# calebhabesh/NM03-Capstone-Project

Hardware: AMD Instinct MI355X
Metric: DICOM slices/sec through full pipeline (T1+C cohort) at 1/2/4/8 MI355X (higher is better)
Workload: dtype fp32

## Files before the change

### include/nm03/engine.h

```cpp
#pragma once

#include <cstdint>
#include <functional>
#include <memory>
#include <string>
#include <vector>

#include "nm03/golden.h"
#include "nm03/params.h"

namespace nm03 {

struct WorkItem {
  std::string path;
  std::string out_dir;
};

enum SliceCode : int32_t {
  kSliceOk = 0,
  kSliceLoadError = 1,
  kSliceTooSmall = 2,
  kSliceDeviceError = 3,
  kSliceExportError = 4,
  kSliceNotRun = 5,
};

struct SliceStatus {
  int32_t code = kSliceNotRun;
  std::string message;
};

struct StageTimes {
  double load_s = 0;
  double h2d_s = 0;
  double kernels_s = 0;
  double write_s = 0;
  double load_cpu_s = 0;
  double write_cpu_s = 0;
  double slot_cpu_s = 0;
  double wall_s = 0;
  int64_t batches = 0, slices_ok = 0, slices_failed = 0;
  int64_t bytes_in = 0, bytes_out = 0;
  int64_t jpeg_fallbacks = 0;
};

struct EngineConfig {
  int device = 0;
  int batch_size = 25;
  int streams = 3;
  int threads = 16;
  std::vector<int> cpus;
  int max_dim = 512;
  PipelineParams pipe;
  RenderParams render;
  bool export_jpeg = true;
  bool resume = false;
  bool host_only = false;
  uint32_t jpeg_out_cap = 0;
  bool shared_stream = false;
  int pack_slack = -1;
  int upload_chunk_kb = -1;
  int create_writers = 4;
  bool lazy_slots = false;
};

// ... 46 lines not shown
```

### include/nm03/gpu_types.h

```cpp
#pragma once

#include <cstdint>

namespace nm03::gpu {

inline constexpr int kMedTileW = 64, kMedTileH = 64;
inline constexpr int kShpTileW = 64, kShpTileH = 64;
inline constexpr int kSrgMaxDim = 512;
inline constexpr int kMaxSliceDim = 4096;

constexpr uint32_t xcd_tile(uint32_t b, uint32_t n) {
  const uint32_t x = b & 7u, k = b >> 3, q = n >> 3, r = n & 7u;
  return (x < r ? x * (q + 1u) : r * (q + 1u) + (x - r) * q) + k;
}

struct SliceDesc {
  uint32_t raw_off;
  uint32_t mask_off;
  uint16_t w, h;
  uint16_t wpr;
  uint8_t type;
  uint8_t stored_bits;
  float slope, intercept;
  uint32_t seed_off;
  uint16_t seed_count;
  uint16_t flags;
  uint32_t f32_off;
  uint32_t med_tile0;
  uint32_t blob_off;
  uint32_t lut_off;
  uint32_t lut_base;
};
static_assert(sizeof(SliceDesc) == 52, "SliceDesc layout");
inline constexpr uint32_t kNoLut = 0xFFFFFFFFu;
inline constexpr uint16_t kSliceFlagPacked12 = 1;

struct TileDesc {
  uint32_t slice;
  uint16_t tx, ty;
};

struct SeedXY {
  int16_t x, y;
};

struct SliceStats {
  uint32_t key_min, key_max;
  uint32_t s_min, s_max;
};

struct PipeConsts {
  float nmin, nmax, nlow, nhigh, cmin, cmax;
  float gain;
  float band_lo, band_hi;
  float taps[16];
  int mask_radius;
  int median_k;
  int connectivity;
// ... 45 lines not shown
```

### include/nm03/pack12.h

```cpp
#pragma once

#include <cstddef>
#include <cstdint>

namespace nm03::pack12 {

bool available();

size_t pack(const uint16_t* src, size_t n, uint8_t* dst);

bool fits12(const uint16_t* src, size_t n);

void pack_stream(const uint16_t* src, size_t n, uint8_t* dst);

bool pack_stream_checked(const uint16_t* src, size_t n, uint8_t* dst);

void unpack(const uint8_t* src, size_t n, uint16_t* dst);

}
```

### src/io/pack12.cpp

```cpp
#include "nm03/pack12.h"

#include <immintrin.h>

#include <cstdlib>
#include <cstring>

#include "nm03/dicom.h"

namespace nm03::pack12 {

namespace {

__attribute__((target("avx2"))) size_t pack_avx2(const uint16_t* src, size_t n, uint8_t* dst) {
  __m256i acc = _mm256_setzero_si256();
  for (size_t i = 0; i < n; i += 16) acc = _mm256_or_si256(acc, _mm256_loadu_si256(reinterpret_cast<const __m256i*>(src + i)));
  if (!_mm256_testz_si256(acc, _mm256_set1_epi16((short)0xF000))) return 0;
  const __m256i lo_mask = _mm256_set1_epi32(0x00000FFF), hi_mask = _mm256_set1_epi32(0x00FFF000);
  const __m256i shuf = _mm256_setr_epi8(0, 1, 2, 4, 5, 6, 8, 9, 10, 12, 13, 14, -1, -1, -1, -1,
                                        0, 1, 2, 4, 5, 6, 8, 9, 10, 12, 13, 14, -1, -1, -1, -1);
  uint8_t* d = dst;
  for (size_t i = 0; i < n; i += 16, d += 24) {
    const __m256i v = _mm256_loadu_si256(reinterpret_cast<const __m256i*>(src + i));
    const __m256i p = _mm256_or_si256(_mm256_and_si256(v, lo_mask), _mm256_and_si256(_mm256_srli_epi32(v, 4), hi_mask));
    const __m256i c = _mm256_shuffle_epi8(p, shuf);
// ... 60 lines not shown
    }
    if (m32 < m) {
      acc = _mm512_or_si512(acc, _mm512_zextsi256_si512(_mm256_loadu_si256(reinterpret_cast<const __m256i*>(src + i + m32))));
      pack16(src + i + m32, bounce + m32 / 2 * 3);
    }
    bounce_out(dst + i / 2 * 3, bounce, m / 2 * 3);
  }
  _mm_sfence();
  return _mm512_test_epi16_mask(acc, _mm512_set1_epi16((short)0xF000)) == 0;
}

bool use_avx512() {
  static const bool ok = [] {
    return __builtin_cpu_supports("avx512f") && __builtin_cpu_supports("avx512bw") &&
           __builtin_cpu_supports("avx512vbmi");
  }();
  return ok;
}

bool pack_stream_any(const uint16_t* src, size_t n, uint8_t* dst) {
  return use_avx512() ? pack_stream_avx512(src, n, dst) : pack_stream_avx2(src, n, dst);
}

}

bool fits12(const uint16_t* src, size_t n) { return n && !(n & 15) && available() && fits_avx2(src, n); }

void pack_stream(const uint16_t* src, size_t n, uint8_t* dst) { (void)pack_stream_any(src, n, dst); }

bool pack_stream_checked(const uint16_t* src, size_t n, uint8_t* dst) {
  return n && !(n & 15) && available() && pack_stream_any(src, n, dst);
}

bool available() {
  static const bool ok = __builtin_cpu_supports("avx2");
  return ok;
}

size_t pack(const uint16_t* src, size_t n, uint8_t* dst) {
  if (n == 0 || (n & 15) || !available()) return 0;
  return pack_avx2(src, n, dst);
}

void unpack(const uint8_t* src, size_t n, uint16_t* dst) {
  for (size_t k = 0; 2 * k < n; ++k) {
    const uint32_t v = (uint32_t)src[3 * k] | ((uint32_t)src[3 * k + 1] << 8) | ((uint32_t)src[3 * k + 2] << 16);
// ... 7 lines not shown
```

### src/kernels/k1_median.hip

```cpp
#include <hip/hip_runtime.h>

#include <cstdlib>

#include "device_util.h"
#include "nm03/gpu_types.h"
#include "nm03/kernels.h"
#include "nm03/pixel_math.h"

namespace nm03::gpu {
using nm03::gpu::vmax;
using nm03::gpu::vmin;
#include "nm03/median_net.inc"

template <int K>
__device__ __forceinline__ void run_net(const uint32_t* P, int stride, int r, int g, u16x2* out) {
  auto ld = [&](int rr, int cc) -> u16x2 { return as_u16x2(P[(r + rr) * stride + 8 * g + cc]); };
  if constexpr (K == 3) median_net_k3_w8_h1<u16x2>(ld, out);
  else if constexpr (K == 5) median_net_k5_w8_h1<u16x2>(ld, out);
  else if constexpr (K == 7) median_net_k7_w8_h1<u16x2>(ld, out);
  else median_net_k9_w8_h1<u16x2>(ld, out);
}

template <int K>
__global__ __launch_bounds__(256) __attribute__((amdgpu_waves_per_eu(K <= 7 ? 4 : 2))) void median_kernel(const uint16_t* __restrict__ raw, uint16_t* __restrict__ med,
                                                     const SliceDesc* __restrict__ descs,
                                                     const TileDesc* __restrict__ tiles, SliceStats* stats,
                                                     uint32_t* __restrict__ tile_mm, int dbg,
                                                     const uint16_t* __restrict__ blob, uint16_t* __restrict__ raw_out) {
  constexpr int R = K / 2;
  constexpr int PW = 32 + K - 1;
  constexpr int PS = PW | 1;
  constexpr int PR = 64 + K - 1;
  __shared__ uint32_t P[PR * PS];

  const TileDesc t = tiles[blockIdx.x];
  const SliceDesc d = descs[t.slice];
  const int x0 = t.tx * kMedTileW, y0 = t.ty * kMedTileH;
  const int W = d.w, H = d.h;
  const bool from_blob = blob != nullptr;
  const bool packed = from_blob && (d.flags & kSliceFlagPacked12);
  const uint16_t* src = from_blob ? blob + d.blob_off : raw + d.raw_off;
  const uint8_t* pb = reinterpret_cast<const uint8_t*>(src);
  auto sample = [&](int y, int x) -> uint16_t {
    const uint32_t p = (uint32_t)y * W + x;
    if (!packed) return src[p];
    const uint32_t o = (3u * p) >> 1;
    const uint32_t v = (uint32_t)pb[o] | ((uint32_t)pb[o + 1] << 8);
    return (uint16_t)((p & 1u) ? (v >> 4) : (v & 0xFFFu));
  };
  uint16_t* rdst = from_blob ? raw_out + d.raw_off : nullptr;
  const int yin_hi = min(y0 + kMedTileH, H), xin_hi = min(x0 + kMedTileW, W);

  uint32_t kmin = 0xFFFFu, kmax = 0u;
  const uint32_t ksb = d.stored_bits;
  const uint32_t km = d.type == kI16 ? 1u << (ksb - 1u) : 0u, kc = d.type == kI16 ? 0x8000u - km : 0u;
  auto key_pair = [&](uint32_t lo, uint32_t hi) -> uint32_t {
    const uint32_t a = (__builtin_amdgcn_ubfe(lo, 0u, ksb) ^ km) + kc;
    const uint32_t b = (__builtin_amdgcn_ubfe(hi, 0u, ksb) ^ km) + kc;
    return __builtin_amdgcn_perm(b, a, 0x05040100u);
  };
  u16x2 pmin = as_u16x2(0xFFFFFFFFu), pmax = as_u16x2(0u);
  if ((W & 3) == 0 && (d.raw_off & 3) == 0 && (!from_blob || packed || (d.blob_off & 3) == 0)) {
    constexpr int NT = (PR * 10 + 255) / 256;
    uint2 ld[NT][2];
#pragma unroll
    for (int t = 0; t < NT; ++t) {
      const int i = threadIdx.x + 256 * t;
      if (i >= PR * 10) break;
      const int r = i / 10, gi = i - r * 10;
      const int y = clampi(y0 - R + r, 0, H - 1);
#pragma unroll
      for (int h = 0; h < 2; ++h) {
        const int xs = clampi(x0 - 4 + 4 * (gi + 8 * h), 0, W - 4);
        if (packed) {
          const size_t o = ((size_t)y * W + xs) * 3 >> 1;
          ld[t][h] = *reinterpret_cast<const uint2*>(pb + (o & ~(size_t)3));
        } else {
          ld[t][h] = *reinterpret_cast<const uint2*>(src + (size_t)y * W + xs);
        }
      }
    }
#pragma unroll
    for (int t = 0; t < NT; ++t) {
      const int i = threadIdx.x + 256 * t;
      if (i >= PR * 10) break;
      const int r = i / 10, gi = i - r * 10;
      const int yy = y0 - R + r;
      const int y = clampi(yy, 0, H - 1);
      const bool row_in = rdst && yy >= y0 && yy < yin_hi;
      uint16_t px[2][4];
#pragma unroll
      for (int h = 0; h < 2; ++h) {
        const int g4 = gi + 8 * h;
        const int xs = x0 - 4 + 4 * g4;
        uint2 v = ld[t][h];
        if (packed) {
          const size_t o = ((size_t)y * W + clampi(xs, 0, W - 4)) * 3 >> 1;
          const uint64_t b = ((uint64_t)v.x | ((uint64_t)v.y << 32)) >> ((o & 2) * 8);
          v.x = ((uint32_t)b & 0xFFFu) | (((uint32_t)(b >> 12) & 0xFFFu) << 16);
          v.y = ((uint32_t)(b >> 24) & 0xFFFu) | (((uint32_t)(b >> 36) & 0xFFFu) << 16);
        }
        px[h][0] = (uint16_t)v.x;
        px[h][1] = (uint16_t)(v.x >> 16);
        px[h][2] = (uint16_t)v.y;
        px[h][3] = (uint16_t)(v.y >> 16);
        if (xs < 0) px[h][1] = px[h][2] = px[h][3] = px[h][0];
        if (xs >= W) px[h][0] = px[h][1] = px[h][2] = px[h][3];
        const bool store = h == 0 ? gi >= 1 : (g4 >= 10 && g4 <= 16);
        if (store && row_in && xs >= x0 && xs < xin_hi) {
          typedef unsigned int u32x2 __attribute__((ext_vector_type(2)));
          __builtin_nontemporal_store(u32x2{v.x, v.y}, reinterpret_cast<u32x2*>(rdst + (size_t)yy * W + xs));
        }
      }
#pragma unroll
      for (int q = 0; q < 4; ++q) {
        const int c = 4 * gi + q - (4 - R);
        if (c < 0 || c >= PW) continue;
        const uint32_t kp = key_pair(px[0][q], px[1][q]);
        P[r * PS + c] = kp;
// ... 111 lines not shown
```

### src/python/bindings.cpp

```cpp
#include <hip/hip_runtime_api.h>
#include <pybind11/functional.h>
#include <pybind11/numpy.h>
#include <pybind11/pybind11.h>
#include <pybind11/stl.h>

#include <sys/mman.h>
#include <unistd.h>

#include <algorithm>
#include <chrono>
#include <cstring>
#include <mutex>
#include <thread>
#include <vector>

#include "nm03/app.h"
#include "nm03/cohort.h"
#include "nm03/comm.h"
#include "nm03/cpu_sampler.h"
#include "nm03/dicom.h"
#include "nm03/engine.h"
#include "nm03/metaimage.h"
#include "nm03/numa.h"
#include "nm03/golden.h"
#include "nm03/jpeg.h"
#include "nm03/jpeg_dct.h"
#include "nm03/jpeg_lossless.h"
#include "nm03/kernels.h"
#include "nm03/synth.h"
#include "nm03/volume.h"
#include "nm03/volume_slabs.h"

namespace py = pybind11;
using namespace nm03;

namespace {

template <class T>
py::array_t<T> to_np(const std::vector<T>& v, std::vector<py::ssize_t> shape) {
  py::array_t<T> a(shape);
  std::memcpy(a.mutable_data(), v.data(), v.size() * sizeof(T));
  return a;
}

template <class T>
std::vector<T> from_np(const py::array_t<T, py::array::c_style | py::array::forcecast>& a) {
// ... 489 lines not shown
        s.rows = rows;
        s.cols = cols;
        s.seed = seed;
        s.threads = threads;
        s.test_slice = test_slice;
        s.decoy_series = decoy;
        s.type = signed_px ? kI16 : kU16;
        py::gil_scoped_release nogil;
        return synth::generate_cohort(s);
      },
      py::arg("data_root"), py::arg("patients") = 20, py::arg("min_slices") = 21, py::arg("max_slices") = 25,
      py::arg("rows") = 256, py::arg("cols") = 256, py::arg("seed") = 20250404, py::arg("threads") = 8,
      py::arg("test_slice") = true, py::arg("decoy") = false, py::arg("signed") = false);
  m.def("synth_flat", [](const std::string& root, int count, int rows, int cols, uint64_t seed, int threads) {
    py::gil_scoped_release nogil;
    return synth::generate_flat(root, count, rows, cols, seed, threads);
  });
  m.def("phantom_slice", [](int rows, int cols, int patient, int slice, int nslices, uint64_t seed) {
    std::vector<uint16_t> v((size_t)rows * cols);
    synth::phantom_slice(rows, cols, patient, slice, nslices, seed, v.data());
    return to_np<uint16_t>(v, {rows, cols});
  });

  m.def(
      "golden_run",
      [](py::array_t<uint16_t, py::array::c_style | py::array::forcecast> raw, const std::string& type, int stored_bits,
         float slope, float intercept, const PipelineParams& p, const RenderParams& rp, float sx, float sy) {
        golden::SliceInput s = slice_from(raw, type, stored_bits, slope, intercept, sx, sy);
        golden::SliceResult r = golden::run(s, p, true);
        py::dict d;
        d["clipped"] = to_np<float>(r.clipped, {s.h, s.w});
        d["median"] = to_np<float>(r.median, {s.h, s.w});
        d["sharpened"] = to_np<float>(r.sharpened, {s.h, s.w});
        d["band"] = mask2d(r.band, s.h, s.w);
        d["region"] = mask2d(r.region, s.h, s.w);
        d["eroded"] = mask2d(r.eroded, s.h, s.w);
        d["dilated"] = mask2d(r.dilated, s.h, s.w);
        d["window"] = py::make_tuple(r.window_lo, r.window_hi);
        golden::SliceJpegs j = golden::export_jpegs(s, r, p, rp);
        d["jpeg_original"] = py::bytes((const char*)j.original.data(), j.original.size());
        d["jpeg_processed"] = py::bytes((const char*)j.processed.data(), j.processed.size());
        if (rp.overlay) {
          d["overlay"] = to_np<uint8_t>(j.overlay_canvas, {rp.out_height, rp.out_width, 3});
          d["jpeg_overlay"] = py::bytes((const char*)j.overlay.data(), j.overlay.size());
        }
        return d;
// ... 158 lines not shown
            }
            return w;
          },
          py::arg("data_root"), py::arg("out_root"), py::arg("reaper") = nullptr);
  struct Ticket {
    RunTicket t;
  };
  py::class_<Ticket>(m, "RunTicket");
  auto times_dict = [](const StageTimes& t) {
    py::dict td;
    td["load_s"] = t.load_s;
    td["h2d_s"] = t.h2d_s;
    td["kernels_s"] = t.kernels_s;
    td["write_s"] = t.write_s;
    td["load_cpu_s"] = t.load_cpu_s;
    td["write_cpu_s"] = t.write_cpu_s;
    td["slot_cpu_s"] = t.slot_cpu_s;
    td["wall_s"] = t.wall_s;
    td["batches"] = t.batches;
    td["slices_ok"] = t.slices_ok;
    td["slices_failed"] = t.slices_failed;
    td["bytes_in"] = t.bytes_in;
    td["bytes_out"] = t.bytes_out;
    td["jpeg_fallbacks"] = t.jpeg_fallbacks;
    return td;
  };
  auto compact = [times_dict](const std::vector<SliceStatus>& st, const StageTimes& t) {
    py::array_t<int32_t> codes((py::ssize_t)st.size());
    auto c = codes.mutable_unchecked<1>();
    py::dict msgs;
    for (size_t i = 0; i < st.size(); ++i) {
      c((py::ssize_t)i) = st[i].code;
      if (st[i].code != kSliceOk) msgs[py::int_(i)] = st[i].message;
    }
    return py::make_tuple(codes, msgs, times_dict(t));
  };
  py::class_<Engine>(m, "Engine")
      .def(py::init<const EngineConfig&>())
      .def(
          "run",
          [times_dict](Engine& e, const std::vector<std::pair<std::string, std::string>>& items) {
            std::vector<WorkItem> wi;
            for (auto& p : items) wi.push_back({p.first, p.second});
            StageTimes t;
            std::vector<SliceStatus> st;
            {
// ... 765 lines not shown
```

### src/runtime/engine.cpp

```cpp
#include "nm03/engine.h"

#include <hip/hip_runtime_api.h>
#include <fcntl.h>
#include <linux/capability.h>
#include <signal.h>
#include <sys/mman.h>
#include <sys/prctl.h>
#include <sys/resource.h>
#include <sys/syscall.h>
#include <unistd.h>

#include <algorithm>
#include <ctime>
#include <atomic>
#include <array>
#include <chrono>
#include <condition_variable>
#include <cstdlib>
#include <cstring>
#include <deque>
#include <unordered_map>
#include <mutex>
#include <tuple>
#include <thread>
// ... 17 lines not shown
namespace {

constexpr size_t kAlign = 256;
inline size_t align_up(size_t v, size_t a) { return (v + a - 1) / a * a; }
inline int64_t thread_cpu_ns() {
  timespec ts;
  clock_gettime(CLOCK_THREAD_CPUTIME_ID, &ts);
  return (int64_t)ts.tv_sec * 1000000000 + ts.tv_nsec;
}

inline double now_s() {
  return std::chrono::duration<double>(std::chrono::steady_clock::now().time_since_epoch()).count();
}

enum Plane { kPBand = 0, kPRegion, kPDilated, kPEroded, kPBorderR, kPBorderE, kPBorderD, kNumPlanes };

struct LoadedSlice {
  bool ok = false;
  int w = 0, h = 0;
  uint8_t type = kU16, stored_bits = 16;
  float slope = 1.f, intercept = 0.f, sx = 1.f, sy = 1.f;
  uint32_t blob_off = 0;
  bool packed = false;
};


struct Slot {
  hipStream_t stream = nullptr;
  hipEvent_t ev0 = nullptr, ev1 = nullptr, ev2 = nullptr;
  hipStream_t up = nullptr;
  bool owns_stream = true;
  int cap_slices = 0, cap_canvases = 0;
  size_t cap_pixels = 0;
  size_t hole_slack = 0;
  std::atomic<size_t> hole_credit{0};
  size_t off_stats = 0, off_desc = 0, off_medt = 0, off_shpt = 0, off_seeds = 0, off_render = 0, off_jpeg = 0,
         raw_base = 0, blob_bytes = 0;
  size_t max_medt = 0, max_shpt = 0;
  uint8_t* h_blob = nullptr;
  uint8_t* raw_cpu = nullptr;
  uint8_t* h_single = nullptr;
  size_t single_bytes = 0;
  uint8_t* d_blob = nullptr;
  uint16_t* d_raw_x = nullptr;
  uint16_t* d_med = nullptr;
  uint32_t* d_tile_mm = nullptr;
// ... 127 lines not shown
  }
  hipStream_t s = nullptr;
  check_hip(hipStreamCreateWithFlags(&s, hipStreamNonBlocking), what);
  return s;
}

template <class T>
T* dmalloc(size_t count, const char* what) {
  void* p = nullptr;
  check_hip(hipMalloc(&p, std::max<size_t>(count, 1) * sizeof(T)), what);
  return (T*)p;
}

}

struct Engine::Impl {
  EngineConfig cfg;
  numa::Placement place;
  std::unique_ptr<ThreadPool> pool;
  std::vector<std::unique_ptr<Slot>> slots;
  std::vector<uint8_t> jpeg_header;
  int32_t divs[64];
  PipeConsts pc{};
  bool pack12_ = pack12::available();
  uint32_t out_cap_ = 0;
  bool host_only_ = false;
  std::vector<uint8_t> tmpl_[2];

  explicit Impl(const EngineConfig& c) : cfg(c), place(c.device, c.cpus) {
    if (const char* e = std::getenv("NM03_PACK12"); e && *e && *e == '0') pack12_ = false;
    out_cap_ = cfg.jpeg_out_cap ? std::max<uint32_t>(64, cfg.jpeg_out_cap)
                                : (uint32_t)std::max<size_t>(32 * 1024, (size_t)cfg.render.out_width * cfg.render.out_height * 3 / 8) + 64;
    out_cap_ = (out_cap_ + 15u) & ~15u;
    overlay_ = cfg.render.overlay;
    if (overlay_ && cfg.host_only)
      throw std::invalid_argument("overlay is rendered and encoded on the GPU: not available with host_only");
    if (overlay_ && cfg.render.jpeg_sampling == jpeg::kSamplingGray)
      throw std::invalid_argument("overlay needs a YCbCr JPEG layout (jpeg_sampling 0 or 1): a gray file cannot carry colour");
    ov_cap_ = cfg.jpeg_out_cap ? out_cap_ : (2 * (out_cap_ - 64) + 64 + 15u) & ~15u;
    ov_color_ = (uint32_t)cfg.render.overlay_color[0] | ((uint32_t)cfg.render.overlay_color[1] << 8) |
                ((uint32_t)cfg.render.overlay_color[2] << 16);
    upload_chunk_ = cfg.upload_chunk_kb < 0 ? (size_t)2 << 20 : (size_t)cfg.upload_chunk_kb << 10;
    host_only_ = cfg.host_only;
    if (host_only_) upload_chunk_ = 0;
    if (cfg.batch_size < 1) cfg.batch_size = 1;
    if (cfg.streams < 1) cfg.streams = 1;
    if (cfg.max_dim < 16) cfg.max_dim = 16;
    if (cfg.max_dim > kMaxSliceDim) throw DeviceError("max_dim above " + std::to_string(kMaxSliceDim) + " not supported");
    const auto& p = cfg.pipe;
    if (p.median_window != 3 && p.median_window != 5 && p.median_window != 7 && p.median_window != 9)
      throw DeviceError("median window must be 3, 5, 7 or 9");
    if (p.sharpen_mask < 1 || p.sharpen_mask > 15 || !(p.sharpen_mask & 1))
      throw DeviceError("sharpen mask must be odd and ≤ 15");
// ... 398 lines not shown
        if (e == hipSuccess) return;
        if (e != hipErrorNotReady) check_hip(e, "batch sync");
        if (now_s() > until) break;
        for (int k = 0; k < 32; ++k) __builtin_ia32_pause();
      }
    }
    const double scale = (double)std::max(1, nslices);
    const double target = 0.8 * s.batch_ema_s * scale;
    for (;;) {
      const hipError_t e = hipEventQuery(ev);
      if (e == hipSuccess) break;
      if (e != hipErrorNotReady) check_hip(e, "batch sync");
      const double ahead = target - (now_s() - t_enq);
      if (ahead > 100e-6)
        std::this_thread::sleep_for(std::chrono::duration<double>(std::min(ahead, 250e-6)));
      else
        std::this_thread::sleep_for(std::chrono::microseconds(20));
    }
    const double took = (now_s() - t_enq) / scale;
    s.batch_ema_s = s.batch_ema_s > 0 ? 0.75 * s.batch_ema_s + 0.25 * took : took;
  }

  void load_into(Slot& s, int i, size_t item, const std::string& path, SliceStatus& st, std::atomic<int64_t>& load_ns,
                 std::atomic<int64_t>& bytes_in) {
    thread_local std::vector<uint8_t> buf;
    TraceRange tr("nm03.load");
    const double t0 = now_s();
    try {
      if (fault_plan().corrupt_dicom == (int64_t)item) throw SliceError("injected fault: corrupt DICOM data");
      dicom::SliceFile file(AT_FDCWD, path.c_str(), path, dicom::ReadMode::kStaged);
      const dicom::Header& h = file.header(buf);
      const int frame = dicom::select_frame(h, cfg.pipe.frame);
      const size_t n = file.size();
      const int md = cfg.pipe.min_dim;
      if (md > 0 && (h.cols < md || h.rows < md)) {
        st.code = kSliceTooSmall;
        st.message = "Image dimensions too small: " + std::to_string(h.cols) + "x" + std::to_string(h.rows);
      } else if (h.cols > cfg.max_dim || h.rows > cfg.max_dim) {
        st.code = kSliceLoadError;
        st.message = "Image dimensions " + std::to_string(h.cols) + "x" + std::to_string(h.rows) +
                     " exceed the engine limit " + std::to_string(cfg.max_dim);
      } else {
        const size_t npix = (size_t)h.rows * h.cols;
        const uint16_t* samples = pack12_ ? file.staged_samples(frame) : nullptr;
        const size_t plen = align_up(npix / 4 * 3, 8), ulen = align_up(npix, 8);
        const bool packable = samples && pack12::available() && (npix & 15) == 0;
        const size_t cap = s.cap_pixels + s.hole_slack;
        size_t idx = 0, off = 0;
        bool packed = false, reserved = false, credit = false;
        auto reserve = [&](size_t len) {
          uint64_t w = s.alloc_word.load(std::memory_order_relaxed);
          for (;;) {
            const size_t used = (size_t)(w & Slot::kUsedMask), n = (size_t)(w >> Slot::kAllocShift);
            if (used + len > cap) throw SliceError("batch pixel capacity exceeded");
            if (n >= s.max_allocs) throw SliceError("batch allocation table full");
            const uint64_t nw = ((uint64_t)(n + 1) << Slot::kAllocShift) | (uint64_t)(used + len);
            if (s.alloc_word.compare_exchange_weak(w, nw, std::memory_order_acq_rel, std::memory_order_relaxed)) {
              idx = n;
              off = used;
              break;
            }
          }
          s.allocs[idx].off = off;
          s.allocs[idx].len = len;
          reserved = true;
        };
        try {
          const bool low12 = h.bits_stored <= 12;
          if (packable && !low12) {
            size_t c = s.hole_credit.load(std::memory_order_relaxed);
            while (c >= plen && !s.hole_credit.compare_exchange_weak(c, c - plen, std::memory_order_acq_rel)) {
            }
            credit = c >= plen;
          }
          if (credit) {
            reserve(plen);
            uint8_t* dst = reinterpret_cast<uint8_t*>(reinterpret_cast<uint16_t*>(s.raw_cpu) + off);
            packed = pack12::pack_stream_checked(samples, npix, dst);
            if (packed) {
              s.hole_credit.fetch_add(plen, std::memory_order_acq_rel);
            } else {
              uint64_t last = ((uint64_t)(idx + 1) << Slot::kAllocShift) | (uint64_t)(off + plen);
              const uint64_t grown = ((uint64_t)(idx + 1) << Slot::kAllocShift) | (uint64_t)(off + ulen);
              if (off + ulen <= cap &&
                  s.alloc_word.compare_exchange_strong(last, grown, std::memory_order_acq_rel, std::memory_order_relaxed)) {
                s.allocs[idx].len = ulen;
                s.hole_credit.fetch_add(plen, std::memory_order_acq_rel);
              } else {
                s.allocs[idx].done.store(true, std::memory_order_release);
                reserve(ulen);
              }
              file.pixels16(reinterpret_cast<uint16_t*>(s.raw_cpu) + off, frame);
            }
          } else {
            packed = packable && (low12 || pack12::fits12(samples, npix));
            reserve(packed ? plen : ulen);
            uint16_t* dst = reinterpret_cast<uint16_t*>(s.raw_cpu) + off;
            if (packed) {
              pack12::pack_stream(samples, npix, reinterpret_cast<uint8_t*>(dst));
            } else {
              file.pixels16(dst, frame);
            }
          }
        } catch (...) {
          if (reserved) s.allocs[idx].done.store(true, std::memory_order_release);
          throw;
        }
        s.allocs[idx].done.store(true, std::memory_order_release);
        LoadedSlice& L = s.loaded[i];
        L.w = h.cols;
        L.h = h.rows;
        L.type = h.type == kU8 ? kU16 : h.type;
        L.stored_bits = (uint8_t)(h.type == kU8 ? 8 : h.bits_stored);
        L.slope = cfg.pipe.apply_rescale ? h.slope : 1.f;
        L.intercept = cfg.pipe.apply_rescale ? h.intercept : 0.f;
        L.sx = h.spacing_x;
        L.sy = h.spacing_y;
        L.blob_off = (uint32_t)off;
        L.packed = packed;
        L.ok = true;
        st.code = kSliceOk;
        bytes_in += (int64_t)n;
      }
    } catch (const std::exception& e) {
      st.code = kSliceLoadError;
      st.message = e.what();
    }
    load_ns += (int64_t)((now_s() - t0) * 1e9);
  }

  bool outputs_exist(const WorkItem& w) const {
    const std::string base = cohort::with_slash(w.out_dir) + cohort::stem(w.path);
    return access((base + "_original.jpg").c_str(), F_OK) == 0 && access((base + "_processed.jpg").c_str(), F_OK) == 0 &&
           (!overlay_ || access((base + "_overlay.jpg").c_str(), F_OK) == 0);
  }

  static inline thread_local std::vector<Seed> seeds_cache_;
  static inline thread_local int seeds_w_ = 0, seeds_h_ = 0;
  void build_and_run(Slot& s, int mode, StageTimes* acc, BatchMark* mark = nullptr) {
    const int nl = (int)s.live.size();
    uint8_t* hb = s.h_blob;
    auto* stats = reinterpret_cast<SliceStats*>(hb + s.off_stats);
    auto* desc = reinterpret_cast<SliceDesc*>(hb + s.off_desc);
    auto* medt = reinterpret_cast<TileDesc*>(hb + s.off_medt);
    auto* shpt = reinterpret_cast<TileDesc*>(hb + s.off_shpt);
    auto* seeds = reinterpret_cast<SeedXY*>(hb + s.off_seeds);
    auto* rd = reinterpret_cast<RenderDesc*>(hb + s.off_render);
    auto* jd = reinterpret_cast<JpegDesc*>(hb + s.off_jpeg);
    int nmed = 0, nshp = 0, nseed = 0, ncanv = 0;
    s.any_canvas = false;
    uint32_t mask_off = 0;
    s.max_w = s.max_h = 0;
    const int cw = cfg.render.out_width, ch = cfg.render.out_height;
    const uint32_t canvas_bytes = (uint32_t)(cw * ch);
    const uint8_t fill = opacity_u8(cfg.render.label_opacity), bval = opacity_u8(cfg.render.border_opacity);
    uint32_t xoff = 0;
    for (int c = 0; c < nl; ++c) {
      const LoadedSlice& L = s.loaded[s.live[c]];
      stats[c] = SliceStats{0xFFFFFFFFu, 0u, 0xFFFFFFFFu, 0u};
      SliceDesc& d = desc[c];
      std::memset(&d, 0, sizeof(d));
      const uint32_t raw_off = xoff;
      xoff += (uint32_t)align_up((size_t)L.w * L.h, 8);
      d.raw_off = raw_off;
      d.blob_off = L.blob_off;
      d.flags = L.packed ? kSliceFlagPacked12 : 0;
      d.w = (uint16_t)L.w;
      d.h = (uint16_t)L.h;
      d.wpr = (uint16_t)((L.w + 63) / 64);
      d.mask_off = mask_off;
      mask_off += (uint32_t)(d.h * d.wpr);
      d.type = L.type;
      d.stored_bits = L.stored_bits;
      d.slope = L.slope;
      d.intercept = L.intercept;
      std::tie(d.lut_off, d.lut_base) = norm_lut(L.type, L.stored_bits, L.slope, L.intercept, s.stream);
      d.f32_off = raw_off;
      if (L.w != seeds_w_ || L.h != seeds_h_) {
        seeds_cache_ = reference_seeds(L.w, L.h);
        seeds_w_ = L.w;
        seeds_h_ = L.h;
      }
      const auto& sv = seeds_cache_;
      d.seed_off = (uint32_t)nseed;
      d.seed_count = (uint16_t)std::min<size_t>(sv.size(), kMaxSeeds);
      for (int k = 0; k < d.seed_count; ++k) seeds[nseed++] = SeedXY{(int16_t)sv[k].x, (int16_t)sv[k].y};
      d.med_tile0 = (uint32_t)nmed;
      for (int ty = 0; ty < (L.h + kMedTileH - 1) / kMedTileH; ++ty)
        for (int tx = 0; tx < (L.w + kMedTileW - 1) / kMedTileW; ++tx) medt[nmed++] = TileDesc{(uint32_t)c, (uint16_t)tx, (uint16_t)ty};
// ... 176 lines not shown
    fallback = jpeg::encode_scan_rgb(rgb.data(), cw, ch, 3 * cw, t, (jpeg::Sampling)cfg.render.jpeg_sampling);
    if (fallbacks) ++*fallbacks;
    return false;
  }

  static int small_batch_spin(size_t count) { return count <= 16 ? 200 : 0; }
  void process_batch(Slot& s, const std::vector<WorkItem>& items, const IoDirs& dirs, size_t batch, uint64_t prio,
                     size_t first, size_t count, std::vector<SliceStatus>& status, StageTimes& acc,
                     std::mutex& acc_m, const std::function<void(size_t)>& on_start, BatchMark* mark = nullptr) {
    if (mark) mark->claim = now_s();
    s.loaded.assign(count, LoadedSlice{});
    if (!s.allocs) {
      s.max_allocs = 2 * (size_t)s.cap_slices;
      s.allocs.reset(new Slot::Alloc[s.max_allocs]);
    }
    for (size_t k = 0; k < s.max_allocs; ++k) s.allocs[k].done.store(false, std::memory_order_relaxed);
    s.alloc_word.store(0, std::memory_order_relaxed);
    s.hole_credit.store(s.hole_slack, std::memory_order_relaxed);
    s.uploaded = 0;
    s.upload_started = false;
    s.loads_finished.store(0, std::memory_order_relaxed);
    s.wake_at.store(0, std::memory_order_relaxed);
    s.progress_quiet.store(false, std::memory_order_relaxed);
    std::atomic<int64_t> load_ns{0}, bytes_in{0}, write_ns{0}, bytes_out{0}, load_cpu_ns{0}, write_cpu_ns{0};
    std::string upload_error;
    {
      TaskGroup tg(*pool);
      tg.for_each(
          count,
          [&](size_t i) {
            if (on_start) on_start(first + i);
            if (cfg.resume && outputs_exist(items[first + i])) {
              status[first + i] = SliceStatus{kSliceOk, "resumed: outputs already present"};
            } else {
              load_into(s, (int)i, first + i, items[first + i].path, status[first + i], load_ns, bytes_in);
            }
            if (upload_chunk_) {
              const size_t lf = s.loads_finished.fetch_add(1, std::memory_order_seq_cst) + 1;
              if (!s.progress_quiet.load(std::memory_order_relaxed) &&
                  (lf >= s.wake_at.load(std::memory_order_seq_cst) || lf == count) &&
                  s.prog_waiting.load(std::memory_order_seq_cst)) {
                { std::lock_guard<std::mutex> g(s.prog_m); }
                s.prog_cv.notify_one();
              }
            }
          },
          2 * prio, &load_cpu_ns);
      if (upload_chunk_) {
        try {
          upload_progress(s, count);
        } catch (const std::exception& e) {
          upload_error = e.what();
        }
      }
      tg.wait(small_batch_spin(count));
    }
    if (mark) mark->loaded = now_s();
    s.live.clear();
// ... 93 lines not shown
                const uint8_t* seg = use_ofb[c] ? ofb[c].data() : s.h_ov_out + c * (size_t)ov_cap_;
                const size_t len = use_ofb[c] ? ofb[c].size() : (size_t)s.h_ov_sizes[c];
                jpeg::write_jpeg_at(AT_FDCWD, std::string(), base + "_overlay.jpg", jpeg_header, seg, len,
                                    &dirs.creating[dirs.out_dir[item]]);
                bytes_out += (int64_t)(jpeg_header.size() + len + 2);
              }
            } catch (const std::exception& e) {
              status[item] = SliceStatus{kSliceExportError, std::string("Error in export stage: ") + e.what()};
            }
            write_ns += (int64_t)((now_s() - t0) * 1e9);
          },
          2 * prio + 1, &write_cpu_ns, creates ? cfg.create_writers : 0);
      tg.wait(small_batch_spin(count));
    }
    if (mark) mark->end = now_s();
    std::lock_guard<std::mutex> g(acc_m);
    acc.load_s += load_ns.load() * 1e-9;
    acc.write_s += write_ns.load() * 1e-9;
    acc.load_cpu_s += load_cpu_ns.load() * 1e-9;
    acc.write_cpu_s += write_cpu_ns.load() * 1e-9;
    acc.h2d_s += local.h2d_s;
    acc.kernels_s += local.kernels_s;
    acc.bytes_in += bytes_in.load();
    acc.bytes_out += bytes_out.load();
    acc.jpeg_fallbacks += fallbacks;
    acc.batches += 1;
  }

  static std::vector<std::pair<size_t, size_t>> plan_batches(size_t n, size_t B) {
    std::vector<std::pair<size_t, size_t>> out;
    if (n == 0 || B == 0) return out;
    const size_t k = (n + B - 1) / B, q = n / k, rem = n % k;
    size_t first = 0;
    for (size_t b = 0; b < k; ++b) {
      const size_t len = q + (b < rem ? 1 : 0);
      out.push_back({first, len});
      first += len;
    }
    return out;
  }

  struct Job {
    std::shared_ptr<const std::vector<WorkItem>> items;
    std::unique_ptr<IoDirs> dirs;
    std::function<void(size_t)> on_start;
    std::vector<SliceStatus> status;
// ... 335 lines not shown
```

Before: 465,400.

## Add adaptive per-group bit-width packing for host-to-device slice upload

Adds an adaptive packer that splits each slice into groups of 32 samples, each stored at 0, 6, 8, 12 or 16 bits, with a directory entry for every 8 groups. The median kernel decodes it in place using the directory. It is used by default for slices of at least 512x512 samples whose width is a multiple of 32, and only when the packed size is smaller than the raw size. The aim is to cut the bytes staged and copied over PCIe. In exchange it adds CPU packing work plus a staging copy per slice, and extra directory loads and bit extraction in the median kernel.

```diff
diff --git a/include/nm03/engine.h b/include/nm03/engine.h
--- a/include/nm03/engine.h
+++ b/include/nm03/engine.h
@@ -41,6 +41,7 @@
   double wall_s = 0;
   int64_t batches = 0, slices_ok = 0, slices_failed = 0;
   int64_t bytes_in = 0, bytes_out = 0;
+  int64_t bytes_blob = 0;
   int64_t jpeg_fallbacks = 0;
 };
 
diff --git a/include/nm03/gpu_types.h b/include/nm03/gpu_types.h
--- a/include/nm03/gpu_types.h
+++ b/include/nm03/gpu_types.h
@@ -34,6 +34,7 @@
 static_assert(sizeof(SliceDesc) == 52, "SliceDesc layout");
 inline constexpr uint32_t kNoLut = 0xFFFFFFFFu;
 inline constexpr uint16_t kSliceFlagPacked12 = 1;
+inline constexpr uint16_t kSliceFlagAdaptive = 2;
 
 struct TileDesc {
   uint32_t slice;
diff --git a/include/nm03/pack12.h b/include/nm03/pack12.h
--- a/include/nm03/pack12.h
+++ b/include/nm03/pack12.h
@@ -17,4 +17,21 @@
 
 void unpack(const uint8_t* src, size_t n, uint16_t* dst);
 
+inline constexpr size_t kGroup = 32;
+inline constexpr size_t kBlockGroups = 8;
+
+inline constexpr size_t adaptive_dir_bytes(size_t n) { return (n / kGroup + kBlockGroups - 1) / kBlockGroups * 8; }
+inline constexpr size_t adaptive_max_bytes(size_t n) { return adaptive_dir_bytes(n) + 2 * n; }
+inline constexpr size_t adaptive_stage_bytes(size_t n) { return adaptive_max_bytes(n) + 64; }
+
+enum AdaptiveIsa : int { kIsaScalar = 0, kIsaAvx2 = 1, kIsaAvx512 = 2 };
+bool adaptive_isa_available(int isa);
+
+size_t pack_adaptive(const uint16_t* src, size_t n, unsigned stored_bits, uint8_t* stage);
+size_t pack_adaptive_isa(int isa, const uint16_t* src, size_t n, unsigned stored_bits, uint8_t* stage);
+
+void adaptive_commit(uint8_t* dst, const uint8_t* stage, size_t bytes);
+
+void unpack_adaptive(const uint8_t* src, size_t n, uint16_t* dst);
+
 }
diff --git a/src/io/pack12.cpp b/src/io/pack12.cpp
--- a/src/io/pack12.cpp
+++ b/src/io/pack12.cpp
@@ -106,6 +106,183 @@
   return use_avx512() ? pack_stream_avx512(src, n, dst) : pack_stream_avx2(src, n, dst);
 }
 
+
+inline unsigned code_of(unsigned or_of_samples) {
+  return or_of_samples == 0 ? 0u : or_of_samples < 64u ? 3u : or_of_samples < 256u ? 4u : or_of_samples < 4096u ? 6u : 8u;
+}
+
+struct DirWriter {
+  uint8_t* base;
+  uint8_t* p;
+  uint64_t entry = 0;
+  size_t g = 0;
+  explicit DirWriter(uint8_t* dst, size_t n) : base(dst), p(dst + adaptive_dir_bytes(n)) {}
+  inline void open() {
+    if ((g & 7) == 0) entry = (uint64_t)((size_t)(p - base) >> 3);
+  }
+  inline void close(unsigned code) {
+    entry |= (uint64_t)code << (32 + 4 * (g & 7));
+    p += 8 * code;
+    if ((++g & 7) == 0) std::memcpy(base + (g / 8 - 1) * 8, &entry, 8);
+  }
+  inline size_t finish() {
+    if (g & 7) std::memcpy(base + g / 8 * 8, &entry, 8);
+    return (size_t)(p - base);
+  }
+};
+
+size_t pack_adaptive_scalar(const uint16_t* src, size_t n, unsigned mask, uint8_t* dst) {
+  DirWriter w(dst, n);
+  for (size_t i = 0; i < n; i += kGroup) {
+    unsigned m = 0;
+    for (size_t k = 0; k < kGroup; ++k) m |= src[i + k] & mask;
+    const unsigned code = code_of(m), bits = 2 * code;
+    w.open();
+    uint64_t acc = 0;
+    unsigned have = 0;
+    uint8_t* q = w.p;
+    for (size_t k = 0; k < kGroup && bits; ++k) {
+      acc |= (uint64_t)(src[i + k] & mask) << have;
+      have += bits;
+      while (have >= 8) {
+        *q++ = (uint8_t)acc;
+        acc >>= 8;
+        have -= 8;
+      }
+    }
+    w.close(code);
+  }
+  return w.finish();
+}
+
+__attribute__((target("avx2"))) inline void pack16v(__m256i v, uint8_t* d) {
+  const __m256i lo_mask = _mm256_set1_epi32(0x00000FFF), hi_mask = _mm256_set1_epi32(0x00FFF000);
+  const __m256i shuf = _mm256_setr_epi8(0, 1, 2, 4, 5, 6, 8, 9, 10, 12, 13, 14, -1, -1, -1, -1,
+                                        0, 1, 2, 4, 5, 6, 8, 9, 10, 12, 13, 14, -1, -1, -1, -1);
+  const __m256i p = _mm256_or_si256(_mm256_and_si256(v, lo_mask), _mm256_and_si256(_mm256_srli_epi32(v, 4), hi_mask));
+  const __m256i c = _mm256_shuffle_epi8(p, shuf);
+  _mm_storeu_si128(reinterpret_cast<__m128i*>(d), _mm256_castsi256_si128(c));
+  _mm_storeu_si128(reinterpret_cast<__m128i*>(d + 12), _mm256_extracti128_si256(c, 1));
+}
+
+__attribute__((target("avx2"))) size_t pack_adaptive_avx2(const uint16_t* src, size_t n, unsigned mask, uint8_t* dst) {
+  DirWriter w(dst, n);
+  const __m256i vm = _mm256_set1_epi16((short)mask);
+  const __m256i above6 = _mm256_set1_epi16((short)0xFFC0), above8 = _mm256_set1_epi16((short)0xFF00),
+                above12 = _mm256_set1_epi16((short)0xF000);
+  const __m256i m6 = _mm256_set1_epi32(0x3F), m6h = _mm256_set1_epi32(0xFC0);
+  for (size_t i = 0; i < n; i += kGroup) {
+    const __m256i a = _mm256_and_si256(_mm256_loadu_si256(reinterpret_cast<const __m256i*>(src + i)), vm);
+    const __m256i b = _mm256_and_si256(_mm256_loadu_si256(reinterpret_cast<const __m256i*>(src + i + 16)), vm);
+    const __m256i o = _mm256_or_si256(a, b);
+    w.open();
+    unsigned code;
+    if (_mm256_testz_si256(o, above6)) {
+      if (_mm256_testz_si256(o, o)) {
+        code = 0;
+      } else {
+        code = 3;
+        const __m256i ta = _mm256_or_si256(_mm256_and_si256(a, m6), _mm256_and_si256(_mm256_srli_epi32(a, 10), m6h));
+        const __m256i tb = _mm256_or_si256(_mm256_and_si256(b, m6), _mm256_and_si256(_mm256_srli_epi32(b, 10), m6h));
+        pack16v(_mm256_permute4x64_epi64(_mm256_packus_epi32(ta, tb), 0xD8), w.p);
+      }
+    } else if (_mm256_testz_si256(o, above8)) {
+      code = 4;
+      _mm256_storeu_si256(reinterpret_cast<__m256i*>(w.p), _mm256_permute4x64_epi64(_mm256_packus_epi16(a, b), 0xD8));
+    } else if (_mm256_testz_si256(o, above12)) {
+      code = 6;
+      pack16v(a, w.p);
+      pack16v(b, w.p + 24);
+    } else {
+      code = 8;
+      _mm256_storeu_si256(reinterpret_cast<__m256i*>(w.p), a);
+      _mm256_storeu_si256(reinterpret_cast<__m256i*>(w.p + 32), b);
+    }
+    w.close(code);
+  }
+  return w.finish();
+}
+
+__attribute__((target("avx2,avx512f,avx512bw,avx512vbmi"))) size_t pack_adaptive_avx512(const uint16_t* src, size_t n,
+                                                                                         unsigned mask, uint8_t* dst) {
+  DirWriter w(dst, n);
+  alignas(64) static const uint8_t kIdx12[64] = {
+      0,  1,  2,  4,  5,  6,  8,  9,  10, 12, 13, 14, 16, 17, 18, 20, 21, 22, 24, 25, 26, 28,
+      29, 30, 32, 33, 34, 36, 37, 38, 40, 41, 42, 44, 45, 46, 48, 49, 50, 52, 53, 54, 56, 57,
+      58, 60, 61, 62, 0,  0,  0,  0,  0,  0,  0,  0,  0,  0,  0,  0,  0,  0,  0,  0};
+  alignas(64) static const uint8_t kIdx6[64] = {0,  1,  2,  8,  9,  10, 16, 17, 18, 24, 25, 26, 32, 33, 34, 40,
+                                                41, 42, 48, 49, 50, 56, 57, 58, 0,  0,  0,  0,  0,  0,  0,  0};
+  const __m512i idx12 = _mm512_load_si512(kIdx12), idx6 = _mm512_load_si512(kIdx6);
+  const __m512i vm = _mm512_set1_epi16((short)mask);
+  const __m512i above6 = _mm512_set1_epi16((short)0xFFC0), above8 = _mm512_set1_epi16((short)0xFF00),
+                above12 = _mm512_set1_epi16((short)0xF000);
+  const __m512i lo_mask = _mm512_set1_epi32(0x00000FFF), hi_mask = _mm512_set1_epi32(0x00FFF000);
+  for (size_t i = 0; i < n; i += kGroup) {
+    const __m512i v = _mm512_and_si512(_mm512_loadu_si512(src + i), vm);
+    w.open();
+    unsigned code;
+    if (_mm512_test_epi16_mask(v, above6) == 0) {
+      if (_mm512_test_epi16_mask(v, v) == 0) {
+        code = 0;
+      } else {
+        code = 3;
+        const __m512i t = _mm512_or_si512(_mm512_and_si512(v, _mm512_set1_epi32(0x3F)),
+                                          _mm512_and_si512(_mm512_srli_epi32(v, 10), _mm512_set1_epi32(0xFC0)));
+        const __m512i u = _mm512_or_si512(_mm512_and_si512(t, _mm512_set1_epi64(0xFFF)),
+                                          _mm512_and_si512(_mm512_srli_epi64(t, 20), _mm512_set1_epi64(0xFFF000)));
+        _mm512_storeu_si512(w.p, _mm512_permutexvar_epi8(idx6, u));
+      }
+    } else if (_mm512_test_epi16_mask(v, above8) == 0) {
+      code = 4;
+      _mm256_storeu_si256(reinterpret_cast<__m256i*>(w.p), _mm512_cvtepi16_epi8(v));
+    } else if (_mm512_test_epi16_mask(v, above12) == 0) {
+      code = 6;
+      const __m512i p = _mm512_or_si512(_mm512_and_si512(v, lo_mask), _mm512_and_si512(_mm512_srli_epi32(v, 4), hi_mask));
+      _mm512_storeu_si512(w.p, _mm512_permutexvar_epi8(idx12, p));
+    } else {
+      code = 8;
+      _mm512_storeu_si512(w.p, v);
+    }
+    w.close(code);
+  }
+  return w.finish();
+}
+
+}
+
+bool adaptive_isa_available(int isa) {
+  return isa == kIsaScalar || (isa == kIsaAvx2 && available()) || (isa == kIsaAvx512 && use_avx512());
+}
+
+size_t pack_adaptive_isa(int isa, const uint16_t* src, size_t n, unsigned stored_bits, uint8_t* stage) {
+  if (n == 0 || n % kGroup || stored_bits < 1 || stored_bits > 16 || !adaptive_isa_available(isa)) return 0;
+  const unsigned mask = (1u << stored_bits) - 1u;
+  return isa == kIsaAvx512 ? pack_adaptive_avx512(src, n, mask, stage)
+         : isa == kIsaAvx2 ? pack_adaptive_avx2(src, n, mask, stage)
+                           : pack_adaptive_scalar(src, n, mask, stage);
+}
+
+size_t pack_adaptive(const uint16_t* src, size_t n, unsigned stored_bits, uint8_t* stage) {
+  return pack_adaptive_isa(use_avx512() ? kIsaAvx512 : available() ? kIsaAvx2 : kIsaScalar, src, n, stored_bits, stage);
+}
+
+void adaptive_commit(uint8_t* dst, const uint8_t* stage, size_t bytes) { dicom::stream_copy(dst, stage, bytes); }
+
+void unpack_adaptive(const uint8_t* src, size_t n, uint16_t* dst) {
+  for (size_t g = 0; g * kGroup < n; ++g) {
+    uint64_t e;
+    std::memcpy(&e, src + g / kBlockGroups * 8, 8);
+    const unsigned j = g % kBlockGroups;
+    size_t off = (size_t)(uint32_t)e * 8;
+    for (unsigned k = 0; k < j; ++k) off += 8 * ((e >> (32 + 4 * k)) & 15u);
+    const unsigned bits = 2 * (unsigned)((e >> (32 + 4 * j)) & 15u);
+    for (size_t k = 0; k < kGroup && g * kGroup + k < n; ++k) {
+      const size_t bit = k * bits;
+      uint32_t v = 0;
+      for (unsigned b = 0; 8 * b < (bit & 7) + bits; ++b) v |= (uint32_t)src[off + bit / 8 + b] << (8 * b);
+      dst[g * kGroup + k] = (uint16_t)((v >> (bit & 7)) & ((1u << bits) - 1u));
+    }
+  }
 }
 
 bool fits12(const uint16_t* src, size_t n) { return n && !(n & 15) && available() && fits_avx2(src, n); }
diff --git a/src/kernels/k1_median.hip b/src/kernels/k1_median.hip
--- a/src/kernels/k1_median.hip
+++ b/src/kernels/k1_median.hip
@@ -39,6 +39,7 @@
   const int W = d.w, H = d.h;
   const bool from_blob = blob != nullptr;
   const bool packed = from_blob && (d.flags & kSliceFlagPacked12);
+  const bool adaptive = from_blob && (d.flags & kSliceFlagAdaptive);
   const uint16_t* src = from_blob ? blob + d.blob_off : raw + d.raw_off;
   const uint8_t* pb = reinterpret_cast<const uint8_t*>(src);
   auto sample = [&](int y, int x) -> uint16_t {
@@ -60,23 +61,60 @@
     return __builtin_amdgcn_perm(b, a, 0x05040100u);
   };
   u16x2 pmin = as_u16x2(0xFFFFFFFFu), pmax = as_u16x2(0u);
-  if ((W & 3) == 0 && (d.raw_off & 3) == 0 && (!from_blob || packed || (d.blob_off & 3) == 0)) {
+  if (adaptive || ((W & 3) == 0 && (d.raw_off & 3) == 0 && (!from_blob || packed || (d.blob_off & 3) == 0))) {
     constexpr int NT = (PR * 10 + 255) / 256;
     uint2 ld[NT][2];
-#pragma unroll
-    for (int t = 0; t < NT; ++t) {
-      const int i = threadIdx.x + 256 * t;
-      if (i >= PR * 10) break;
-      const int r = i / 10, gi = i - r * 10;
-      const int y = clampi(y0 - R + r, 0, H - 1);
-#pragma unroll
-      for (int h = 0; h < 2; ++h) {
-        const int xs = clampi(x0 - 4 + 4 * (gi + 8 * h), 0, W - 4);
-        if (packed) {
-          const size_t o = ((size_t)y * W + xs) * 3 >> 1;
-          ld[t][h] = *reinterpret_cast<const uint2*>(pb + (o & ~(size_t)3));
-        } else {
-          ld[t][h] = *reinterpret_cast<const uint2*>(src + (size_t)y * W + xs);
+    uint32_t meta[NT][2];
+    if (adaptive) {
+      const uint2* dir = reinterpret_cast<const uint2*>(pb);
+      uint2 de[NT][2];
+#pragma unroll
+      for (int t = 0; t < NT; ++t) {
+        const int i = threadIdx.x + 256 * t;
+        if (i >= PR * 10) break;
+        const int r = i / 10, gi = i - r * 10;
+        const int y = clampi(y0 - R + r, 0, H - 1);
+#pragma unroll
+        for (int h = 0; h < 2; ++h) {
+          const int xs = clampi(x0 - 4 + 4 * (gi + 8 * h), 0, W - 4);
+          de[t][h] = dir[((uint32_t)y * W + xs) >> 8];
+        }
+      }
+#pragma unroll
+      for (int t = 0; t < NT; ++t) {
+        const int i = threadIdx.x + 256 * t;
+        if (i >= PR * 10) break;
+        const int r = i / 10, gi = i - r * 10;
+        const int y = clampi(y0 - R + r, 0, H - 1);
+#pragma unroll
+        for (int h = 0; h < 2; ++h) {
+          const int xs = clampi(x0 - 4 + 4 * (gi + 8 * h), 0, W - 4);
+          const uint32_t p = (uint32_t)y * W + xs, j4 = (p >> 3) & 28u;
+          const uint2 e = de[t][h];
+          const uint32_t below = e.y & ((1u << j4) - 1u), code = (e.y >> j4) & 15u;
+          const uint32_t s2 = (below & 0x0F0F0F0Fu) + ((below >> 4) & 0x0F0F0F0Fu);
+          const uint32_t o = 8u * (e.x + ((s2 * 0x01010101u) >> 24)) + ((p & 31u) >> 2) * code;
+          ld[t][h] = *reinterpret_cast<const uint2*>(pb + (size_t)(o & ~3u));
+          meta[t][h] = code | ((o & 3u) << 4);
+        }
+      }
+    } else {
+#pragma unroll
+      for (int t = 0; t < NT; ++t) {
+        const int i = threadIdx.x + 256 * t;
+        if (i >= PR * 10) break;
+        const int r = i / 10, gi = i - r * 10;
+        const int y = clampi(y0 - R + r, 0, H - 1);
+#pragma unroll
+        for (int h = 0; h < 2; ++h) {
+          const int xs = clampi(x0 - 4 + 4 * (gi + 8 * h), 0, W - 4);
+          if (packed) {
+            const size_t o = ((size_t)y * W + xs) * 3 >> 1;
+            ld[t][h] = *reinterpret_cast<const uint2*>(pb + (o & ~(size_t)3));
+          } else {
+            ld[t][h] = *reinterpret_cast<const uint2*>(src + (size_t)y * W + xs);
+          }
+          meta[t][h] = 0;
         }
       }
     }
@@ -94,7 +132,12 @@
         const int g4 = gi + 8 * h;
         const int xs = x0 - 4 + 4 * g4;
         uint2 v = ld[t][h];
-        if (packed) {
+        if (adaptive) {
+          const uint32_t m = meta[t][h], w = 2u * (m & 15u), msk = (1u << w) - 1u;
+          const uint64_t b = ((uint64_t)v.x | ((uint64_t)v.y << 32)) >> ((m >> 4) * 8u);
+          v.x = ((uint32_t)b & msk) | (((uint32_t)(b >> w) & msk) << 16);
+          v.y = ((uint32_t)(b >> 2u * w) & msk) | (((uint32_t)(b >> 3u * w) & msk) << 16);
+        } else if (packed) {
           const size_t o = ((size_t)y * W + clampi(xs, 0, W - 4)) * 3 >> 1;
           const uint64_t b = ((uint64_t)v.x | ((uint64_t)v.y << 32)) >> ((o & 2) * 8);
           v.x = ((uint32_t)b & 0xFFFu) | (((uint32_t)(b >> 12) & 0xFFFu) << 16);
diff --git a/src/python/bindings.cpp b/src/python/bindings.cpp
--- a/src/python/bindings.cpp
+++ b/src/python/bindings.cpp
@@ -8,6 +8,7 @@
 #include <unistd.h>
 
 #include <algorithm>
+#include <atomic>
 #include <chrono>
 #include <cstring>
 #include <mutex>
@@ -22,6 +23,7 @@
 #include "nm03/engine.h"
 #include "nm03/metaimage.h"
 #include "nm03/numa.h"
+#include "nm03/pack12.h"
 #include "nm03/golden.h"
 #include "nm03/jpeg.h"
 #include "nm03/jpeg_dct.h"
@@ -557,6 +559,52 @@
     return to_np<uint16_t>(v, {rows, cols});
   });
 
+  m.def("adaptive_isa_available", &pack12::adaptive_isa_available);
+  m.def("adaptive_dir_bytes", [](size_t n) { return pack12::adaptive_dir_bytes(n); });
+  m.def("pack_adaptive", [](py::array_t<uint16_t, py::array::c_style | py::array::forcecast> a, unsigned stored_bits, int isa) {
+    const size_t n = (size_t)a.size();
+    std::vector<uint8_t> stage(pack12::adaptive_stage_bytes(n));
+    const size_t bytes = pack12::pack_adaptive_isa(isa, a.data(), n, stored_bits, stage.data());
+    return py::bytes((const char*)stage.data(), bytes);
+  });
+  m.def("unpack_adaptive", [](const std::string& packed, size_t n) {
+    std::vector<uint16_t> out(n);
+    pack12::unpack_adaptive((const uint8_t*)packed.data(), n, out.data());
+    return to_np<uint16_t>(out, {(py::ssize_t)n});
+  });
+  m.def("pack_adaptive_concurrent",
+        [](const std::vector<py::array_t<uint16_t, py::array::c_style | py::array::forcecast>>& slices, unsigned stored_bits,
+           int threads, size_t guard) {
+          size_t cap = 2 * guard;
+          std::vector<std::pair<const uint16_t*, size_t>> in;
+          for (auto& a : slices) {
+            cap += pack12::adaptive_max_bytes((size_t)a.size()) + 16;
+            in.push_back({a.data(), (size_t)a.size()});
+          }
+          std::vector<uint8_t> buf(cap + 16, 0xA5);
+          uint8_t* base = buf.data() + ((16 - ((uintptr_t)buf.data() & 15)) & 15);
+          std::vector<std::pair<size_t, size_t>> where(slices.size());
+          std::atomic<size_t> next{0}, used{guard};
+          {
+            py::gil_scoped_release nogil;
+            std::vector<std::thread> pool;
+            for (int t = 0; t < std::max(threads, 1); ++t)
+              pool.emplace_back([&] {
+                std::vector<uint8_t> stage;
+                for (size_t i; (i = next.fetch_add(1)) < in.size();) {
+                  const size_t n = in[i].second;
+                  stage.resize(pack12::adaptive_stage_bytes(n));
+                  const size_t bytes = pack12::pack_adaptive(in[i].first, n, stored_bits, stage.data());
+                  const size_t off = used.fetch_add((bytes + 15) & ~(size_t)15);
+                  pack12::adaptive_commit(base + off, stage.data(), bytes);
+                  where[i] = {off, bytes};
+                }
+              });
+            for (auto& th : pool) th.join();
+          }
+          return py::make_tuple(py::bytes((const char*)base, cap), where);
+        });
+
   m.def(
       "golden_run",
       [](py::array_t<uint16_t, py::array::c_style | py::array::forcecast> raw, const std::string& type, int stored_bits,
@@ -761,6 +809,7 @@
     td["slices_failed"] = t.slices_failed;
     td["bytes_in"] = t.bytes_in;
     td["bytes_out"] = t.bytes_out;
+    td["bytes_blob"] = t.bytes_blob;
     td["jpeg_fallbacks"] = t.jpeg_fallbacks;
     return td;
   };
diff --git a/src/runtime/engine.cpp b/src/runtime/engine.cpp
--- a/src/runtime/engine.cpp
+++ b/src/runtime/engine.cpp
@@ -63,6 +63,7 @@
   float slope = 1.f, intercept = 0.f, sx = 1.f, sy = 1.f;
   uint32_t blob_off = 0;
   bool packed = false;
+  bool adaptive = false;
 };
 
 
@@ -236,13 +237,18 @@
   std::vector<uint8_t> jpeg_header;
   int32_t divs[64];
   PipeConsts pc{};
+  static constexpr size_t kAdaptiveDefaultMinSamples = 512 * 512;
   bool pack12_ = pack12::available();
+  size_t adaptive_min_ = kAdaptiveDefaultMinSamples;
   uint32_t out_cap_ = 0;
   bool host_only_ = false;
   std::vector<uint8_t> tmpl_[2];
 
   explicit Impl(const EngineConfig& c) : cfg(c), place(c.device, c.cpus) {
-    if (const char* e = std::getenv("NM03_PACK12"); e && *e && *e == '0') pack12_ = false;
+    if (const char* e = std::getenv("NM03_PACK12"); e && *e) {
+      if (*e == '0') pack12_ = false;
+      adaptive_min_ = *e == '2' ? 0 : SIZE_MAX;
+    }
     out_cap_ = cfg.jpeg_out_cap ? std::max<uint32_t>(64, cfg.jpeg_out_cap)
                                 : (uint32_t)std::max<size_t>(32 * 1024, (size_t)cfg.render.out_width * cfg.render.out_height * 3 / 8) + 64;
     out_cap_ = (out_cap_ + 15u) & ~15u;
@@ -687,8 +693,9 @@
   }
 
   void load_into(Slot& s, int i, size_t item, const std::string& path, SliceStatus& st, std::atomic<int64_t>& load_ns,
-                 std::atomic<int64_t>& bytes_in) {
+                 std::atomic<int64_t>& bytes_in, std::atomic<int64_t>& bytes_blob) {
     thread_local std::vector<uint8_t> buf;
+    thread_local std::vector<uint8_t> stage;
     TraceRange tr("nm03.load");
     const double t0 = now_s();
     try {
@@ -712,7 +719,7 @@
         const bool packable = samples && pack12::available() && (npix & 15) == 0;
         const size_t cap = s.cap_pixels + s.hole_slack;
         size_t idx = 0, off = 0;
-        bool packed = false, reserved = false, credit = false;
+        bool packed = false, adaptive = false, reserved = false, credit = false;
         auto reserve = [&](size_t len) {
           uint64_t w = s.alloc_word.load(std::memory_order_relaxed);
           for (;;) {
@@ -732,13 +739,24 @@
         };
         try {
           const bool low12 = h.bits_stored <= 12;
-          if (packable && !low12) {
+          if (samples && npix >= adaptive_min_ && h.cols % (int)pack12::kGroup == 0) {
+            if (stage.size() < pack12::adaptive_stage_bytes(npix)) stage.resize(pack12::adaptive_stage_bytes(npix));
+            const size_t bytes = pack12::pack_adaptive(samples, npix, (unsigned)h.bits_stored, stage.data());
+            const size_t alen = align_up(bytes / 2, 8);
+            if (bytes && alen < ulen) {
+              reserve(alen);
+              pack12::adaptive_commit(reinterpret_cast<uint8_t*>(reinterpret_cast<uint16_t*>(s.raw_cpu) + off), stage.data(), bytes);
+              adaptive = true;
+            }
+          }
+          if (!adaptive && packable && !low12) {
             size_t c = s.hole_credit.load(std::memory_order_relaxed);
             while (c >= plen && !s.hole_credit.compare_exchange_weak(c, c - plen, std::memory_order_acq_rel)) {
             }
             credit = c >= plen;
           }
-          if (credit) {
+          if (adaptive) {
+          } else if (credit) {
             reserve(plen);
             uint8_t* dst = reinterpret_cast<uint8_t*>(reinterpret_cast<uint16_t*>(s.raw_cpu) + off);
             packed = pack12::pack_stream_checked(samples, npix, dst);
@@ -783,9 +801,11 @@
         L.sy = h.spacing_y;
         L.blob_off = (uint32_t)off;
         L.packed = packed;
+        L.adaptive = adaptive;
         L.ok = true;
         st.code = kSliceOk;
         bytes_in += (int64_t)n;
+        bytes_blob += (int64_t)(s.allocs[idx].len * sizeof(uint16_t));
       }
     } catch (const std::exception& e) {
       st.code = kSliceLoadError;
@@ -829,7 +849,7 @@
       xoff += (uint32_t)align_up((size_t)L.w * L.h, 8);
       d.raw_off = raw_off;
       d.blob_off = L.blob_off;
-      d.flags = L.packed ? kSliceFlagPacked12 : 0;
+      d.flags = L.adaptive ? kSliceFlagAdaptive : L.packed ? kSliceFlagPacked12 : 0;
       d.w = (uint16_t)L.w;
       d.h = (uint16_t)L.h;
       d.wpr = (uint16_t)((L.w + 63) / 64);
@@ -1052,7 +1072,7 @@
     s.loads_finished.store(0, std::memory_order_relaxed);
     s.wake_at.store(0, std::memory_order_relaxed);
     s.progress_quiet.store(false, std::memory_order_relaxed);
-    std::atomic<int64_t> load_ns{0}, bytes_in{0}, write_ns{0}, bytes_out{0}, load_cpu_ns{0}, write_cpu_ns{0};
+    std::atomic<int64_t> load_ns{0}, bytes_in{0}, bytes_blob{0}, write_ns{0}, bytes_out{0}, load_cpu_ns{0}, write_cpu_ns{0};
     std::string upload_error;
     {
       TaskGroup tg(*pool);
@@ -1063,7 +1083,7 @@
             if (cfg.resume && outputs_exist(items[first + i])) {
               status[first + i] = SliceStatus{kSliceOk, "resumed: outputs already present"};
             } else {
-              load_into(s, (int)i, first + i, items[first + i].path, status[first + i], load_ns, bytes_in);
+              load_into(s, (int)i, first + i, items[first + i].path, status[first + i], load_ns, bytes_in, bytes_blob);
             }
             if (upload_chunk_) {
               const size_t lf = s.loads_finished.fetch_add(1, std::memory_order_seq_cst) + 1;
@@ -1203,6 +1223,7 @@
     acc.h2d_s += local.h2d_s;
     acc.kernels_s += local.kernels_s;
     acc.bytes_in += bytes_in.load();
+    acc.bytes_blob += bytes_blob.load();
     acc.bytes_out += bytes_out.load();
     acc.jpeg_fallbacks += fallbacks;
     acc.batches += 1;
```

New measurement: 455,900. 2.0% lower.
